# phantomzone-org/fhe-ram

Measured on AMD Instinct MI355X. Metric: encrypted RAM read ops/s + write ops/s at 2^18 entries; achieved HBM GB/s vs peak, higher is better.
Workload: dtype f64

## Files before the change

fhe-ram_amd/csrc/ctx.hpp:

```cpp
#pragma once
#include "../../include/fheram.h"
#include "kernels.hpp"
#include "cmux_chain.hpp"

#include <algorithm>
#include <atomic>
#include <cstdio>
#include <cstdlib>
#include <cstring>
#include <map>
#include <string>
#include <vector>

using namespace fk;

namespace {

thread_local std::string g_create_err;


struct ProfCls {
    uint64_t launches = 0, blocks = 0;
    double ms = 0.0;
    std::vector<std::pair<hipEvent_t, hipEvent_t>> pending;
// ... 128 lines not shown
    unsigned* h_mid_fb = nullptr;
    unsigned* d_mid_sync[2] = {nullptr, nullptr};
    double* d_mid_big[2] = {nullptr, nullptr};
    double* d_mid_y[2] = {nullptr, nullptr};
    uint64_t inv_id[2] = {0, 0};
    double* d_prep_inv = nullptr;
    int32_t* d_ggsw_inv = nullptr;
    hipEvent_t ev_inv[2] = {nullptr, nullptr};
    bool inv_pending[2] = {false, false};
    hipEvent_t ev_wdone = nullptr;
    bool wdone_pending = false;
    hipEvent_t ev_opstart = nullptr;
    bool opstart_valid = false;
    bool wide_unsynced = false;
    bool derive_unsynced = false;
    int32_t* h_pin[2] = {nullptr, nullptr};
    hipEvent_t ev_pin[2] = {nullptr, nullptr};
    int64_t* h_res = nullptr;
    int64_t* d_h_res = nullptr;
    int32_t* h_w = nullptr;
    hipEvent_t ev_w = nullptr;
    bool w_busy = false;
    bool side_begun = false;
    bool trhi_in_C = false;
    bool tree_rotate_pending = false;
    bool words_staged = false;
    int profile = 0;
    std::map<std::string, ProfCls> prof;
    std::vector<hipEvent_t> ev_pool;
    hipEvent_t t0 = nullptr, t1 = nullptr;
// ... 33 lines not shown
}
int check_precision(fheram_ctx* c) {
    if (c->h_ro_flag && __atomic_load_n(c->h_ro_flag, __ATOMIC_RELAXED))
        return fail(c, FHERAM_ERR_PRECISION, "FP64 round-off of an inverse transform exceeded 3/8 (fheram_roundoff_max): the rounded integers are no longer trustworthy");
    return FHERAM_OK;
}
#define HIPCHK(c, call)                                                                     \
    do {                                                                                    \
        hipError_t e_ = (call);                                                             \
        if (e_ != hipSuccess)                                                               \
            return fail((c), FHERAM_ERR_DEVICE, std::string(#call) + ": " + hipGetErrorString(e_)); \
    } while (0)

GlweRef ref(int32_t* p, long sy, long sx) { return GlweRef{p, sy, sx}; }

hipEvent_t get_event(fheram_ctx* c) {
    if (!c->ev_pool.empty()) { hipEvent_t e = c->ev_pool.back(); c->ev_pool.pop_back(); return e; }
    hipEvent_t e = nullptr; c->res.event(&e, true); return e;
}
struct ProfScope {
    fheram_ctx* c; ProfCls* cls = nullptr; hipEvent_t a = nullptr;
    ProfScope(fheram_ctx* c_, const char* name, uint64_t blocks, int steps = 1) : c(c_) {
        if (!c->profile) return;
        if (c->profile == 2 && !strstr(name, "chain_launch")) return;
        cls = &c->prof[name];
        cls->launches += steps; cls->blocks += blocks * steps;
        a = get_event(c);
        hipEventRecord(a, c->cur);
    }
    ~ProfScope() {
// ... 78 lines not shown
            HIPCHK(c, hipMemcpyAsync(c->h_pin[k & 1], src + off, m * sizeof(int32_t), hipMemcpyDeviceToHost, c->stream));
            HIPCHK(c, hipEventRecord(c->ev_pin[k & 1], c->stream));
        }
        if (k > 0) {
            const size_t off = (k - 1) * PIN_CHUNK, m = std::min(PIN_CHUNK, n - off);
            HIPCHK(c, hipEventSynchronize(c->ev_pin[(k - 1) & 1]));
            widen(c->h_pin[(k - 1) & 1], dst + off, m);
        }
    }
    return FHERAM_OK;
}
int stage_words(fheram_ctx* c, int32_t* d_w, const int64_t* w, int n_ct) {
    if (c->w_busy) { HIPCHK(c, hipEventSynchronize(c->ev_w)); c->w_busy = false; }
    const size_t n = (size_t)n_ct * fheram_ctx::GLWE;
    if (!narrow(w, c->h_w, n)) return fail(c, FHERAM_ERR_RANGE, "limb out of the normalised range [-2^16, 2^16]");
    HIPCHK(c, hipMemcpyAsync(d_w, c->h_w, n * sizeof(int32_t), hipMemcpyHostToDevice, c->stream));
    HIPCHK(c, hipEventRecord(c->ev_w, c->stream));
    c->w_busy = true;
    return FHERAM_OK;
}

}
```

fhe-ram_amd/csrc/fheram.hip:

```cpp
#include <unistd.h>
#include <atomic>
#include "path.hpp"

extern "C" {

int fheram_params_default(fheram_params* p) {
    if (!p) return FHERAM_ERR_INVALID_ARG;
    std::memset(p, 0, sizeof(*p));
    p->log_n = 12; p->base2k = 17; p->rank = 1;
    p->k_glwe_pt = 3; p->k_glwe_ct = 51; p->k_ggsw_addr = 68; p->k_evk_trace = 68; p->k_evk_ggsw_inv = 85;
    p->word_size = 4; p->n_decomp = 4;
    p->decomp_n[0] = p->decomp_n[1] = p->decomp_n[2] = p->decomp_n[3] = 3;
    p->max_addr = (uint64_t)1 << 14;
    return FHERAM_OK;
}

const char* fheram_last_error(const fheram_ctx* c) { return c ? c->err.c_str() : g_create_err.c_str(); }

void fheram_config_default(fheram_config* cfg) {
    if (!cfg) return;
    fheram_config d = config_builtin();
    auto env = [](const char* n) { const char* v = getenv(n); return (v && v[0]) ? v[0] : '\0'; };
    if (env("FHERAM_LIMB_SPLIT") == '0') d.limb_split = 0;
    if (env("FHERAM_FINE_SPLIT") == '0') d.fine_split = 0;
// ... 322 lines not shown
    return result_export(c, &run, 1, c->h_res, c->d_h_res, nullptr);
}
int fheram_result_download(fheram_ctx* c, int64_t* out) {
    if (!c || !out) return FHERAM_ERR_INVALID_ARG;
    const int64_t* src = nullptr;
    const int rc = fheram_result_map(c, &src);
    if (rc != FHERAM_OK) return rc;
    std::memcpy(out, src, (size_t)c->ws * fheram_ctx::GLWE * sizeof(int64_t));
    return FHERAM_OK;
}
int fheram_sync(fheram_ctx* c) {
    if (!c) return FHERAM_ERR_INVALID_ARG;
    HIPCHK(c, hipSetDevice(c->device));
    HIPCHK(c, hipStreamSynchronize(c->stream));
    HIPCHK(c, hipGetLastError());
    c->wide_unsynced = c->derive_unsynced = false;
    return check_precision(c);
}
int fheram_roundoff_max(fheram_ctx* c, double* max_out) {
    if (!c || !max_out) return FHERAM_ERR_INVALID_ARG;
    HIPCHK(c, hipSetDevice(c->device));
    HIPCHK(c, hipStreamSynchronize(c->stream));
    HIPCHK(c, hipStreamSynchronize(c->stream2));
    double m = 0.0;
    HIPCHK(c, hipMemcpy(&m, c->d_tw + N, sizeof(double), hipMemcpyDeviceToHost));
    *max_out = m;
    if (c->cfg.monitor && m > MON_LIMIT) __atomic_store_n(c->h_ro_flag, 1u, __ATOMIC_RELAXED);
    return check_precision(c);
}
int fheram_roundoff_reset(fheram_ctx* c) {
    if (!c) return FHERAM_ERR_INVALID_ARG;
// ... 72 lines not shown
    if (w) { rc = fheram_word_stage(c, w, n_w); if (rc != FHERAM_OK) { write_side_abort(c); return rc; } }
    rc = run_op(c, addr, 2, [&] {
        if (!c->side_begun) write_side_begin(o, ctx_view(c));
        int r2 = write_top(o, ctx_view(c));
        return r2 == FHERAM_OK ? write_rows(o, ctx_view(c)) : r2;
    });
    if (rc != FHERAM_OK) return rc;
    c->ram.state = false;
    HIPCHK(c, hipGetLastError());
    return FHERAM_OK;
}

namespace {
int export_glwes(fheram_ctx* c, const int32_t* src, void* dst, int on_device, size_t n_glwe) {
    const size_t n = n_glwe * fheram_ctx::GLWE;
    if (on_device) { HIPCHK(c, hipMemcpyAsync(dst, src, n * 4, hipMemcpyDeviceToDevice, c->stream)); return FHERAM_OK; }
    return download_i64(c, (int64_t*)dst, src, n);
}
int import_glwes(fheram_ctx* c, int32_t* dst, const void* src, int on_device, size_t n_glwe) {
    const size_t n = n_glwe * fheram_ctx::GLWE;
    if (on_device) { HIPCHK(c, hipMemcpyAsync(dst, src, n * 4, hipMemcpyDeviceToDevice, c->stream)); return FHERAM_OK; }
    return upload_i64(c, dst, (const int64_t*)src, n);
}
}

int fheram_shard_info(const fheram_ctx* c, int* shard, int* n_shards, size_t* local_rows) {
    if (!c) return FHERAM_ERR_INVALID_ARG;
    if (shard) *shard = c->shard;
    if (n_shards) *n_shards = c->n_shards;
    if (local_rows) *local_rows = c->rows;
    return FHERAM_OK;
}
int fheram_read_partial(fheram_ctx* c, const fheram_addr* addr, int prepare_write, void* out, int out_on_device) {
    int rc = check_common(c, addr);
    if (rc != FHERAM_OK) return rc;
    if (!out) return fail(c, FHERAM_ERR_INVALID_ARG, "null output");
    if (c->ram.state) return fail(c, FHERAM_ERR_STATE, "invalid call to Memory.read: internal state is true -> requires calling Memory.write");
    HIPCHK(c, hipSetDevice(c->device));
    GlweRef packed;
    rc = read_local(one_addr(c, &addr), ctx_view(c), prepare_write != 0, &packed, true);
    if (rc != FHERAM_OK) return rc;
    HIPCHK(c, hipGetLastError());
    if (prepare_write) c->ram.state = true;
    return export_glwes(c, c->d_part, out, out_on_device, (size_t)c->ws);
}
int fheram_stream_signal(fheram_ctx* c, void* hip_stream) {
    if (!c) return FHERAM_ERR_INVALID_ARG;
    HIPCHK(c, hipSetDevice(c->device));
    HIPCHK(c, hipEventRecord(c->ev_xout, c->stream));
    HIPCHK(c, hipStreamWaitEvent((hipStream_t)hip_stream, c->ev_xout, 0));
    return FHERAM_OK;
}
int fheram_stream_wait(fheram_ctx* c, void* hip_stream) {
    if (!c) return FHERAM_ERR_INVALID_ARG;
    HIPCHK(c, hipSetDevice(c->device));
    HIPCHK(c, hipEventRecord(c->ev_xin, (hipStream_t)hip_stream));
    HIPCHK(c, hipStreamWaitEvent(c->stream, c->ev_xin, 0));
    return FHERAM_OK;
}
int fheram_device_malloc(fheram_ctx* c, size_t bytes, void** out) {
    if (!c || !out || bytes == 0) return fail(c, FHERAM_ERR_INVALID_ARG, "bad argument");
    HIPCHK(c, hipSetDevice(c->device));
    HIPCHK(c, hipMalloc(out, bytes));
    return FHERAM_OK;
}
int fheram_device_free(fheram_ctx* c, void* ptr) {
    if (!c) return FHERAM_ERR_INVALID_ARG;
    HIPCHK(c, hipSetDevice(c->device));
    HIPCHK(c, hipFree(ptr));
    return FHERAM_OK;
}
// ... 143 lines not shown
    return download_i64(c, ggsw_out, c->d_ggsw_tmp, fheram_ctx::GGSW);
}

int fheram_timer_begin(fheram_ctx* c) {
    if (!c) return FHERAM_ERR_INVALID_ARG;
    HIPCHK(c, hipSetDevice(c->device));
    HIPCHK(c, hipEventRecord(c->t0, c->stream));
    return FHERAM_OK;
}
int fheram_timer_end(fheram_ctx* c, float* ms) {
    if (!c || !ms) return FHERAM_ERR_INVALID_ARG;
    HIPCHK(c, hipSetDevice(c->device));
    HIPCHK(c, hipEventRecord(c->t1, c->stream));
    HIPCHK(c, hipEventSynchronize(c->t1));
    HIPCHK(c, hipEventElapsedTime(ms, c->t0, c->t1));
    c->wide_unsynced = c->derive_unsynced = false;
    return check_precision(c);
}
int fheram_profile_enable(fheram_ctx* c, int on) {
    if (!c) return FHERAM_ERR_INVALID_ARG;
    c->profile = on == 2 ? 2 : (on != 0);
    return FHERAM_OK;
}
int fheram_profile_reset(fheram_ctx* c) {
    if (!c) return FHERAM_ERR_INVALID_ARG;
    hipSetDevice(c->device);
    prof_collect(c);
    c->prof.clear();
    return FHERAM_OK;
}
int fheram_profile_get(fheram_ctx* c, const char* cls, uint64_t* launches, uint64_t* blocks, double* total_ms) {
// ... 133 lines not shown
```

fhe-ram_amd/csrc/kernels.hpp:

```cpp
#pragma once
#include "../../include/fheram.h"
#include "fft_dev.hpp"
#include <type_traits>

namespace fk {

#ifdef FK_STAMP
__device__ unsigned long long g_stamps[192];
#define STAMP(i)                                                                                   \
    do {                                                                                           \
        __builtin_amdgcn_sched_barrier(0);                                                         \
        if (threadIdx.x == 0 && blockIdx.x == 0 && blockIdx.y == 0 && blockIdx.z == 0) {           \
            unsigned long long t_;                                                                 \
            asm volatile("s_memtime %0\n\ts_waitcnt lgkmcnt(0)" : "=s"(t_)::"memory");            \
            g_stamps[i] = t_;                                                                      \
        }                                                                                          \
        __builtin_amdgcn_sched_barrier(0);                                                         \
    } while (0)
#define STAMPZ(i)                                                                                  \
    do {                                                                                           \
        __builtin_amdgcn_sched_barrier(0);                                                         \
        if (threadIdx.x == 0 && blockIdx.x == 0 && blockIdx.y == 0 && (blockIdx.z == 0 || blockIdx.z == 3)) { \
            unsigned long long t_;                                                                 \
            asm volatile("s_memtime %0\n\ts_waitcnt lgkmcnt(0)" : "=s"(t_)::"memory");            \
// ... 164 lines not shown
__device__ __forceinline__ void load_ops_p(OpRegs& o, const double* __restrict__ g, int tid) {
#ifdef FK_NO_PROLOGUE_OPS
#pragma unroll
    for (int kk = 0; kk < E / 2; kk++) asm volatile("" : "=v"(o.v[kk].x), "=v"(o.v[kk].y));
#else
    load_ops(o, g, tid);
#endif
}
__device__ __forceinline__ void mac_regs(double (&acc)[E], const double (&x)[E], const OpRegs& o) {
#pragma unroll
    for (int kk = 0; kk < E / 2; kk++) cmac(acc[2 * kk], acc[2 * kk + 1], x[2 * kk], x[2 * kk + 1], o.v[kk].x, o.v[kk].y);
}

constexpr int BF = 3, BI = 1;
#ifndef FK_CHAIN_VGPRS
#define FK_CHAIN_VGPRS 120
#endif
#define FK_WIDE_VGPRS 128
static_assert(BF <= BMAX && BI <= BMAX, "LDS holds BMAX exchange buffers");

template <int S, int R = 0>
__device__ __forceinline__ void fwd_all(double (&x)[S][E], const double* tw, double* data, int tid) {
    if constexpr (R < S) {
        constexpr int C = (S - R < BF) ? (S - R) : BF;
        ntt_fwd<C>(*reinterpret_cast<double(*)[C][E]>(&x[R]), tw, data, tid);
        fwd_all<S, R + C>(x, tw, data, tid);
    }
}

template <int SA, int SG>
__device__ __forceinline__ void ep_mac(double (&acc)[E], const double (&x0)[SA][E], const double (&x1)[SA][E], OpRegs (&g)[SA],
// ... 1196 lines not shown
        const double d1 = take_digit(r_);
        int dst = tid + T * k + ka.t;
        const bool ng = dst >= N;
        if (ng) dst -= N;
        gstore_i32(op + glwe_off(2, co), (unsigned)dst * 4u, cneg((int)d2, ng));
        gstore_i32(op + glwe_off(1, co), (unsigned)dst * 4u, cneg((int)d1, ng));
        gstore_i32(op + glwe_off(0, co), (unsigned)dst * 4u, cneg((int)r_, ng));
    }
}

struct RowChainArgs {
    EpChainArgs ep;
    KsChainArgs ks;
    GlweRef hi, trhi;
    int store_ep = 0;
};
#define FK_READ_CHAIN_ARGS RowChainArgs
#define FK_READ_CHAIN_TABLE 0
#define FK_KS_CHAIN_NAME k_keyswitch_chain
#define FK_READ_CHAIN_NAME k_read_chain
#define FK_VG FK_CHAIN_VGPRS
#include "chain_kernels.inc"
#undef FK_KS_CHAIN_NAME
#undef FK_READ_CHAIN_NAME
#undef FK_VG
#define FK_KS_CHAIN_NAME k_keyswitch_chain_w
#define FK_READ_CHAIN_NAME k_read_chain_w
#define FK_VG FK_WIDE_VGPRS
#include "chain_kernels.inc"
#undef FK_KS_CHAIN_NAME
// ... 803 lines not shown
```

fhe-ram_amd/csrc/launch.hpp:

```cpp
#pragma once
#include "ctx.hpp"

namespace {

template <typename F>
void with_evk(const fheram_ctx* c, F&& f) {
    if (c->s_evk == 5) f(std::integral_constant<int, 5>{});
    else f(std::integral_constant<int, 4>{});
}
template <typename F>
void with_evk_wide(fheram_ctx* c, bool wide, F&& f) {
    if (wide) c->wide_unsynced = true;
    with_evk(c, [&](auto sk) { if (wide) f(sk, std::true_type{}); else f(sk, std::false_type{}); });
}
bool capturing(const fheram_ctx* c) { return c->cfg.graph && !c->profile; }

constexpr int LIMB_SPLIT_MAX = 64;
constexpr int EW_SLICES = 8;
int pick_nco(const fheram_ctx* c, int gx, int gy, bool one_wg = false) {
    if (c->cfg.nco != 0) return c->cfg.nco;
    if (one_wg) return 2;
    return ((long)gx * gy * 2 <= c->cus) ? 1 : 2;
}
void launch_prepare(fheram_ctx* c, const int32_t* in, double* out, int npoly, int64_t gal = 0) {
// ... 16 lines not shown
        hipLaunchKernelGGL((k_ext_product_fine_norm<3, 4>), dim3(gx, gy, 2 * (N / 256)), dim3(256), 0, c->cur, res, big_of(c));
        return;
    }
    if (use_limb_split(c, gx, gy, 4)) {
        hipLaunchKernelGGL((k_ext_product<3, 4, 1, 1>), dim3(gx, gy, 8), dim3(T), LDS_BYTES, c->cur, a, res, ggsw, c->d_tw, big_of(c));
        hipLaunchKernelGGL((k_ext_product<3, 4, 1, 2>), dim3(gx, gy, 2), dim3(T), 0, c->cur, a, res, ggsw, c->d_tw, big_of(c));
        return;
    }
    if (pick_nco(c, gx, gy) == 1) hipLaunchKernelGGL((k_ext_product<3, 4, 1>), dim3(gx, gy, 2), dim3(T), LDS_BYTES, c->cur, a, res, ggsw, c->d_tw, big_of(c));
    else {
        ProfScope pf(c, "ext_product_fused", (uint64_t)gx * gy);
        hipLaunchKernelGGL((k_ext_product<3, 4, 2>), dim3(gx, gy, 1), dim3(T), LDS_BYTES, c->cur, a, res, ggsw, c->d_tw, big_of(c));
    }
}
template <int MODE, int SX, int SK, int SO>
void launch_ks(fheram_ctx* c, const KsArgs& ka, int gx, int gy) {
    if (gx <= 0 || gy <= 0) return;
    ProfScope ps(c, "keyswitch", (uint64_t)gx * gy);
    if (use_fine_split(c, gx, gy, 2 * SK * SX)) {
        KsArgs kb = ka;
        kb.big = big_of(c);
        hipLaunchKernelGGL((k_keyswitch_fine<MODE, SX, SK>), dim3(gx, gy, 2 * SK * SX), dim3(T), LDS_BYTES, c->cur, kb);
        hipLaunchKernelGGL((k_keyswitch_norm<MODE, SX, SK, SO, SX>), dim3(gx, gy, 2 * (N / 256)), dim3(256), 0, c->cur, kb);
        return;
    }
    if (use_limb_split(c, gx, gy, SK)) {
        KsArgs kb = ka;
        kb.big = big_of(c);
        hipLaunchKernelGGL((k_keyswitch<MODE, SX, SK, SO, 1, 1>), dim3(gx, gy, 2 * SK), dim3(T), LDS_BYTES, c->cur, kb);
        hipLaunchKernelGGL((k_keyswitch_norm<MODE, SX, SK, SO>), dim3(gx, gy, 2 * (N / 256)), dim3(256), 0, c->cur, kb);
        return;
    }
    constexpr bool FUSABLE = (SX == 3) && (MODE != KS_PAIR);
    if constexpr (MODE == KS_PAIR && SX == 3 && SO == 3) {
        if (c->cfg.pair_z) {
            hipLaunchKernelGGL((k_pair_z<SK>), dim3(gx, gy, 2), dim3(T), LDS_BYTES, c->cur, ka);
            return;
        }
    }
    if (!FUSABLE || pick_nco(c, gx, gy) == 1) {
        hipLaunchKernelGGL((k_keyswitch<MODE, SX, SK, SO, 1>), dim3(gx, gy, 2), dim3(T), LDS_BYTES, c->cur, ka);
// ... 212 lines not shown
    ra.hi = dst; ra.trhi = dst;
    if (t.ws > 0) {
        c->wide_unsynced = true;
        with_evk(c, [&](auto sk) {
            constexpr int SK = decltype(sk)::value;
            hipLaunchKernelGGL((k_read_chain_t<SK, 4>), dim3(gx, gy, 1), dim3(T), LDS_BYTES, c->cur, with_table(ra, t));
        });
        return;
    }
    with_evk_wide(c, c->wide, [&](auto sk, auto w) {
        constexpr int SK = decltype(sk)::value;
        if constexpr (decltype(w)::value) hipLaunchKernelGGL((k_read_chain_w<SK, 4>), dim3(gx, gy, 1), dim3(T), LDS_BYTES, c->cur, ra);
        else hipLaunchKernelGGL((k_read_chain<SK, 4>), dim3(gx, gy, 1), dim3(T), LDS_BYTES, c->cur, ra);
    });
}
void launch_write_chain(fheram_ctx* c, GlweRef src, int rot_mul, int rot_base, GlweRef data, GlweRef trhi, const double* prep, int d, int n_tr, int gx, int gy, const OpndTable& t) {
    ProfScope ps(c, "write_chain_launch", (uint64_t)gx * gy, 1);
    RowChainArgs ra;
    fill_row_chain(c, ra, prep, d, 0, n_tr);
    ra.ks.base = ks_args(c, src, src, data, trace_key(c, 0), c->gal[0], 0, rot_mul, rot_base);
    ra.ks.buf[0] = ra.ks.buf[1] = data;
    ra.hi = data; ra.trhi = trhi;
    ra.ep.src = data; ra.ep.buf[0] = ra.ep.buf[1] = data;
    c->wide_unsynced = true;
    with_evk(c, [&](auto sk) {
        constexpr int SK = decltype(sk)::value;
        if (t.ws > 0) hipLaunchKernelGGL((k_write_chain_t<SK, 4>), dim3(gx, gy, 1), dim3(T), LDS_BYTES, c->cur, with_table(ra, t));
        else hipLaunchKernelGGL((k_write_chain<SK, 4>), dim3(gx, gy, 1), dim3(T), LDS_BYTES, c->cur, ra);
    });
}
void launch_trace_tail(fheram_ctx* c, GlweRef src, const GlweRef (&b)[2], int start, int n, int gx, int gy,
                       const double* prep = nullptr, int d = 0, GlweRef ep_out = GlweRef{nullptr, 0, 0}, bool store_ep = false, const OpndTable& t = {}) {
    ProfScope ps(c, "keyswitch", (uint64_t)gx * gy, n);
    ProfScope pt(c, "keyswitch_tail_launch", (uint64_t)gx * gy * n, 1);
    TailArgs ta;
    ta.src = src; ta.buf[0] = b[0]; ta.buf[1] = b[1]; ta.tw = c->d_tw; ta.big = big_of(c); ta.sync = c->d_tail_sync;
    ta.n_ep = prep ? d : 0; ta.ep_out = ep_out;
    for (int i = 0; i < TAIL_EP_MAX; i++) ta.ggsw[i] = (prep && i < d) ? prep + (size_t)i * fheram_ctx::GGSW : nullptr;
// ... 87 lines not shown
        }
        live = std::min<size_t>(live, (size_t)h);
        cur = nxt;
    }
    return cur;
}
int coord_first_digit(const fheram_ctx* c, int ci) { int s = 0; for (int i = 0; i < ci; i++) s += (int)c->base2d[i].size(); return s; }
double* digits_of(const fheram_ctx* c, double* table, int ci) { return table + (size_t)coord_first_digit(c, ci) * fheram_ctx::GGSW; }
void coordinate_prepare(fheram_ctx* c, const fheram_addr* addr, int ci, double* table) {
    const int d = (int)c->base2d[ci].size();
    launch_prepare(c, addr->d_ggsw + (size_t)coord_first_digit(c, ci) * fheram_ctx::GGSW, digits_of(c, table, ci), d * (int)(fheram_ctx::GGSW / N));
}
void coordinate_prepare_all(fheram_ctx* c, const fheram_addr* addr, double* table) {
    launch_prepare(c, addr->d_ggsw, table, c->n_digits * (int)(fheram_ctx::GGSW / N));
}
void ggsw_inverse(fheram_ctx* c, const int32_t* in, int32_t* tmp, int d) {
    const long g4 = (long)fheram_ctx::GLWE4;
    int32_t* inp = const_cast<int32_t*>(in);
    KsArgs ka = ks_args(c, ref(inp, (long)fheram_ctx::GGSW, 2 * g4), ref(inp, 0, 0), ref(tmp, (long)fheram_ctx::GGSW, 2 * g4), c->d_atk_inv, -1);
    launch_ks<KS_AUTO, 4, 5, 4>(c, ka, fheram_ctx::DNUM_CT, d);
    KsArgs kt = ks_args(c, ref(tmp, (long)fheram_ctx::GGSW, 2 * g4), ref(tmp, 0, 0), ref(tmp + g4, (long)fheram_ctx::GGSW, 2 * g4), c->d_tsk, 1);
    launch_ks<KS_TENSOR, 4, 5, 4>(c, kt, fheram_ctx::DNUM_CT, d);
}
void coordinate_prepare_inv(fheram_ctx* c, const fheram_addr* addr, int ci, int32_t* tmp, double* prep) {
    const int d = (int)c->base2d[ci].size();
    ggsw_inverse(c, addr->d_ggsw + (size_t)coord_first_digit(c, ci) * fheram_ctx::GGSW, tmp, d);
    launch_prepare(c, tmp, prep, d * (int)(fheram_ctx::GGSW / N));
}

void precompute_inverse(fheram_ctx* c, const fheram_addr* addr, int ci, bool fork, unsigned gate_seq = 0) {
    if (fork && c->wdone_pending) {
        hipStreamWaitEvent(c->stream2, c->ev_wdone, 0);
        c->wdone_pending = false;
    }
    if (fork && gate_seq) {
        if (c->opstart_valid) { hipStreamWaitEvent(c->stream2, c->ev_opstart, 0); c->opstart_valid = false; }
        hipLaunchKernelGGL(k_tail_gate, dim3(1), dim3(64), 0, c->stream2, c->d_tail_sync + TAIL_GROUPS * 32 + 2, gate_seq);
    } else if (fork) {
        hipEventRecord(c->ev_fork, c->stream);
        hipStreamWaitEvent(c->stream2, c->ev_fork, 0);
    }
    hipStream_t keep = c->cur;
    c->cur = c->stream2;
    coordinate_prepare_inv(c, addr, ci, c->d_ggsw_inv + (size_t)coord_first_digit(c, ci) * fheram_ctx::GGSW, digits_of(c, c->d_prep_inv, ci));
    hipEventRecord(c->ev_inv[ci], c->stream2);
    c->cur = keep;
    c->inv_id[ci] = addr->id;
    c->inv_pending[ci] = true;
}
void wait_inverse(fheram_ctx* c, hipStream_t s, int ci) { if (!capturing(c)) hipStreamWaitEvent(s, c->ev_inv[ci], 0); }

}
```

fhe-ram_amd/csrc/path.hpp:

```cpp
#pragma once
#include "launch.hpp"

namespace {

struct Opnds {
    fheram_ctx* c;
    RamState* st;
    const fheram_addr* const* addrs;
    int n, ws;
    double *tab, *tab_inv;
    long stride;
    unsigned src_map;
    bool bank;
    int member(int k) const { return (int)((src_map >> (4 * k)) & 15u); }
    int Y() const { return n * ws; }
    double* prep(int k, int ci) const { return digits_of(c, tab + k * stride, ci); }
    double* inv(int k, int ci) const { return digits_of(c, tab_inv + k * stride, ci); }
    GlweRef slice(GlweRef r, int k) const { r.p += (long)k * ws * r.sy; return r; }
    GlweRef rows(GlweRef r, int k) const { return slice(r, member(k)); }
    OpndTable table() const { return n == 1 ? OpndTable{} : OpndTable{ws, stride, src_map}; }
    bool row_fuse(int d, int n_tr, int gx) const { return use_row_fuse(c, d, n_tr, gx, Y(), bank); }
};
Opnds one_addr(fheram_ctx* c, const fheram_addr* const* a, int ws, RamState* st) { return Opnds{c, st, a, 1, ws, c->d_prep, c->d_prep_inv, 0, 0, false}; }
Opnds one_addr(fheram_ctx* c, const fheram_addr* const* a) { return one_addr(c, a, c->ws, &c->ram); }
// ... 10 lines not shown
}

void read_local_done(const fheram_ctx* c, RamState* st, bool prepare_write) {
    if (c->n2 == 2) st->memo_alone = (prepare_write && c->cfg.memo) ? LOGN - ilog2_ceil(c->rows_glob) : 0;
}
void read_top_done(fheram_ctx* c, RamState* st, bool prepare_write) {
    st->memo_top = prepare_write && c->cfg.memo;
    st->res_in_trtop = st->memo_top;
    c->prep1_ready = false;
}
void write_done(fheram_ctx* c, RamState* st) { st->memo_top = false; st->memo_alone = 0; c->side_begun = false; c->tree_rotate_pending = false; }

template <typename F>
int run_op(fheram_ctx* c, const fheram_addr* addr, int which, F&& enqueue) {
    if (!capturing(c)) return enqueue();
    fheram_addr* a = const_cast<fheram_addr*>(addr);
    const unsigned sig = 1u | (c->ram.memo_top ? 2u : 0u) | ((unsigned)c->ram.memo_alone << 2) | (c->side_begun ? 64u : 0u) |
                         (c->inv_id[0] == addr->id ? 128u : 0u) | (c->inv_id[1] == addr->id ? 256u : 0u);
    if (a->graph[which] && a->graph_sig[which] != sig) { hipGraphExecDestroy(a->graph[which]); a->graph[which] = nullptr; }
    if (!a->graph[which]) {
        hipGraph_t g = nullptr;
        HIPCHK(c, hipStreamBeginCapture(c->stream, hipStreamCaptureModeThreadLocal));
        const int rc = enqueue();
        const hipError_t e = hipStreamEndCapture(c->stream, &g);
        if (rc != FHERAM_OK || e != hipSuccess) {
            if (g) hipGraphDestroy(g);
            return rc != FHERAM_OK ? rc : fail(c, FHERAM_ERR_DEVICE, std::string("hipStreamEndCapture: ") + hipGetErrorString(e));
        }
        const hipError_t e2 = hipGraphInstantiate(&a->graph[which], g, nullptr, nullptr, 0);
        hipGraphDestroy(g);
// ... 7 lines not shown
}

int check_common(fheram_ctx* c, const fheram_addr* addr) {
    if (!c) return FHERAM_ERR_INVALID_ARG;
    mid_rearm(c);
    if (!addr || addr->ctx != c) return fail(c, FHERAM_ERR_INVALID_ARG, "address does not belong to this context (layout mismatch, ram.rs:404)");
    if (addr->empty) return fail(c, FHERAM_ERR_INVALID_ARG, "empty address: fheram_address_alloc without fheram_address_derive");
    if (!c->ram.initialized) return fail(c, FHERAM_ERR_UNINITIALIZED, "unitialized memory: self.data.len()=0");
    if (!c->keys_loaded) return fail(c, FHERAM_ERR_KEYS, "evaluation keys not loaded");
    return FHERAM_OK;
}

int read_local(const Opnds& o, const RamView& a, bool prepare_write, GlweRef* packed_out, bool to_part) {
    fheram_ctx* c = o.c;
    const int n = o.n, ws = o.ws, Y = o.Y(), R = (int)c->rows;
    c->wide = !prepare_write || n > 1;
    if (n == 1 && prepare_write && c->cfg.pre_inv == 1 && !capturing(c) && (c->wide_unsynced || c->derive_unsynced)) {
        hipEventRecord(c->ev_opstart, c->stream);
        c->opstart_valid = true;
    }
    const long G = (long)fheram_ctx::GLWE;
    const long sy = (long)c->rows * G;
    GlweRef data = ref(a.rows, sy, G), A = ref(a.A, sy, G), B = ref(a.B, sy, G);
    GlweRef part = ref(a.part, G, 0);
    const bool all = (c->n_shards == 1 && c->n2 == 2);
    for (int k = 0; k < n; k++)
        if (all) coordinate_prepare_all(c, o.addrs[k], o.tab + k * o.stride); else coordinate_prepare(c, o.addrs[k], 0, o.tab + k * o.stride);
    c->prep1_ready = all;
    read_local_done(c, o.st, prepare_write);
    const int d0 = (int)c->base2d[0].size();
// ... 13 lines not shown
        launch_read_chain(c, data, prepare_write ? &data : nullptr, A, o.prep(0, 0), d0, L0, R, Y, o.table());
        packed = pack_levels(c, a.A, a.A, a.B, sy, G, (size_t)R, Y, 0, L0, keep, a.C, a.D);
    } else {
        for (int k = 0; k < n; k++)
            if (prepare_write) ep_chain(c, o.rows(data, k), o.rows(data, k), o.slice(A, k), o.prep(k, 0), d0, R, ws);
            else ep_chain(c, o.rows(data, k), o.slice(A, k), o.slice(B, k), o.prep(k, 0), d0, R, ws);
        packed = pack_levels(c, prepare_write ? a.rows : a.A, a.A, a.B, sy, G, (size_t)R, Y, L0, L0, keep, a.C, a.D);
    }
    *packed_out = ref(packed, sy, 0);
    if (to_part) launch_copy(c, *packed_out, part, 1, Y);
    return FHERAM_OK;
}
int read_top(const Opnds& o, const RamView& a, bool prepare_write, int32_t* gathered, GlweRef pk) {
    fheram_ctx* c = o.c;
    const int n = o.n, ws = o.ws, Y = o.Y();
    c->wide = !prepare_write || n > 1;
    const long G = (long)fheram_ctx::GLWE;
    GlweRef tmp = ref(a.tmp, G, 0);
    GlweRef last = pk;
    const int d1 = c->n2 == 2 ? (int)c->base2d[1].size() : 0;
    auto tail_top = [&] { return chain_form(c, ChainQuery{false, LOGN, 1, Y}).form == ChainForm::Tail; };
    const bool fuse_ep = c->n2 == 2 && c->cfg.tail_ep && d1 >= 2 && d1 <= TAIL_EP_MAX && tail_top();
    GlweRef ep_out = ref(prepare_write ? a.tree : a.tmp2, G, 0);
    auto products1 = [&] { for (int k = 0; k < n; k++) ep_chain(c, o.slice(pk, k), o.slice(ep_out, k), o.slice(tmp, k), o.prep(k, 1), d1, 1, ws); };
    if (c->n2 == 2) {
        if (gathered) {
            const int kG = ilog2_ceil((size_t)c->n_shards);
            int32_t* a0 = c->d_gat[1];
            int32_t* a1 = c->d_gat[2];
            int32_t* packed = pack_levels(c, gathered, a0, a1, G, (long)ws * G, (size_t)c->n_shards, ws, 0, LOGN - kG);
// ... 77 lines not shown
    return FHERAM_OK;
}
RamView reads_view(const fheram_ctx* c, const ReadBufs& L) { return RamView{c->d_data, L.A, L.B, L.C, nullptr, L.tmp2, L.tmp, L.tmp2, L.res, nullptr, nullptr, nullptr}; }

struct ResRun { const int32_t* src; size_t n; };
int result_export(fheram_ctx* c, const ResRun* runs, int n_runs, int64_t* h, int64_t* d_h, int64_t* out) {
    size_t n = 0;
    for (int i = 0; i < n_runs; i++) {
        const int n4 = (int)(runs[i].n / 4);
        hipLaunchKernelGGL(k_export_i64, dim3((n4 + 255) / 256), dim3(256), 0, c->stream, runs[i].src, reinterpret_cast<long long*>(d_h + n), n4,
                           reinterpret_cast<const long long*>(c->d_tw + N));
        n += runs[i].n;
    }
    HIPCHK(c, hipStreamSynchronize(c->stream));
    HIPCHK(c, hipGetLastError());
    c->wide_unsynced = c->derive_unsynced = false;
    double m;
    std::memcpy(&m, h + n, 8);
    if (c->cfg.monitor && m > MON_LIMIT) __atomic_store_n(c->h_ro_flag, 1u, __ATOMIC_RELAXED);
    const int rc = check_precision(c);
    if (rc == FHERAM_OK && out) std::memcpy(out, h, n * sizeof(int64_t));
    return rc;
}

int reads_export(fheram_ctx* c, const ReadBufs& L, size_t first, size_t n_ct, int64_t* out) {
    const ResRun run{L.res + first * fheram_ctx::GLWE, n_ct * fheram_ctx::GLWE};
    return result_export(c, &run, 1, L.h_res, L.d_h_res, out);
}
template <typename F>
int read_many(fheram_ctx* c, ReadBufs& L, RamState* st, const fheram_addr* const* addrs, int n, int ws, unsigned src_map, bool bank, int64_t* out, F&& kept) {
    int rc = reads_reserve(c, L, n, ws);
    if (rc != FHERAM_OK) return rc;
    const Opnds o = table_opnds(c, st, addrs, n, ws, L.prep, nullptr, src_map, bank);
    rc = read_impl(o, reads_view(c, L), false);
    if (rc != FHERAM_OK) return rc;
    kept(o);
    HIPCHK(c, hipGetLastError());
    return out ? reads_export(c, L, 0, (size_t)n * ws, out) : FHERAM_OK;
}

int write_top(const Opnds& o, const RamView& v) {
    fheram_ctx* c = o.c;
    c->wide = true;
    const long G = (long)fheram_ctx::GLWE;
    const long sy = (long)c->rows * G;
    const int n = o.n, ws = o.ws, Y = o.Y();
    GlweRef wref = ref(v.w, G, 0), tmp = ref(v.tmp, G, 0), tmp2 = ref(v.tmp2, G, 0), tree = ref(v.tree, G, 0);
    GlweRef top = (c->n2 != 1) ? tree : ref(v.rows, sy, 0);
    GlweRef tr = tmp;
    if (o.st->memo_top) tr = ref(v.trtop, G, 0);
    else trace_steps(c, top, tmp, tmp2, 0, LOGN, 1, Y);
    {
        ProfScope ps(c, "elementwise", Y);
        hipLaunchKernelGGL((k_sub_add_norm<3>), dim3(1, Y, EW_SLICES), dim3(256), 0, c->cur, top, tr, wref, top);
    }
    o.st->memo_top = false;
    if (c->n2 == 2) {
// ... 2 lines not shown
            if (n == 1 && c->inv_pending[1]) wait_inverse(c, c->stream, 1);
            for (int k = 0; k < n; k++) coordinate_prepare_inv(c, o.addrs[k], 1, c->d_ggsw_tmp, o.inv(k, 1));
        }
        if (n == 1) { c->inv_pending[1] = false; c->inv_id[1] = 0; }
        for (int k = 0; k < n; k++)
            ep_chain(c, o.slice(tree, k), o.slice(ref(v.part, G, 0), k), o.slice(tmp, k), o.inv(k, 1), (int)c->base2d[1].size(), 1, ws);
        c->tree_rotate_pending = true;
    }
    return FHERAM_OK;
}
void write_side_begin(const Opnds& o, const RamView& v) {
    fheram_ctx* c = o.c;
    c->wide = true;
    const long G = (long)fheram_ctx::GLWE;
    const long sy = (long)c->rows * G;
    hipEventRecord(c->ev_fork, c->stream);
    hipStreamWaitEvent(c->stream2, c->ev_fork, 0);
    c->cur = c->stream2;
    if (c->n2 == 2) {
        const int kept = o.st->memo_alone;
        c->trhi_in_C = kept > 0 && (LOGN - kept) % 2 == 1;
        if (kept > 0) trace_steps(c, ref(v.A, sy, G), ref(c->trhi_in_C ? v.C : v.A, sy, G), ref(c->trhi_in_C ? v.A : v.C, sy, G), kept, LOGN, (int)c->rows, o.Y());
        else trace_steps(c, ref(v.rows, sy, G), ref(v.A, sy, G), ref(v.C, sy, G), 0, LOGN, (int)c->rows, o.Y());
        o.st->memo_alone = 0;
    }
    if (o.n == 1 && c->inv_id[0] == o.addrs[0]->id) wait_inverse(c, c->stream2, 0);
    else for (int k = 0; k < o.n; k++) coordinate_prepare_inv(c, o.addrs[k], 0, c->d_ggsw_tmp2, o.inv(k, 0));
    if (o.n == 1) { c->inv_id[0] = 0; c->inv_pending[0] = false; }
    hipEventRecord(c->ev_join, c->stream2);
    c->cur = c->stream;
    c->side_begun = true;
}
void write_side_abort(fheram_ctx* c) {
    if (!c->side_begun) return;
    hipStreamWaitEvent(c->stream, c->ev_join, 0);
    c->side_begun = false;
}
int write_rows(const Opnds& o, const RamView& v) {
    fheram_ctx* c = o.c;
    c->wide = true;
    const long G = (long)fheram_ctx::GLWE;
    const long sy = (long)c->rows * G;
    const int n = o.n, ws = o.ws, Y = o.Y(), R = (int)c->rows;
    GlweRef data = ref(v.rows, sy, G), A = ref(v.A, sy, G), B = ref(v.B, sy, G), D = ref(v.D, sy, G);
    GlweRef trhi = ref(c->trhi_in_C ? v.C : v.A, sy, G), part = ref(v.part, G, 0);
    const int d0 = (int)c->base2d[0].size();
    const bool fuse = c->n2 == 2 && o.row_fuse(d0, LOGN, R);
    if (fuse) {
        hipStreamWaitEvent(c->stream, c->ev_join, 0);
        launch_write_chain(c, part, c->n_shards, c->shard, data, trhi, o.inv(0, 0), d0, LOGN, R, Y, o.table());
    } else if (c->n2 == 2)
        trace_steps(c, part, B, D, 0, LOGN, R, Y, c->n_shards, c->shard);
    if (c->tree_rotate_pending) {
        ProfScope ps(c, "elementwise", Y);
        hipLaunchKernelGGL((k_rotate<3>), dim3(1, Y, EW_SLICES), dim3(256), 0, c->cur, part, ref(v.tree, G, 0), -(int)c->rows_glob);
    }
    if (!fuse) {
        hipStreamWaitEvent(c->stream, c->ev_join, 0);
        if (c->n2 == 2) {
            ProfScope ps(c, "elementwise", (uint64_t)R * Y);
            hipLaunchKernelGGL((k_sub_add_norm<3>), dim3(R, Y, EW_SLICES), dim3(256), 0, c->cur, data, trhi, B, data);
        }
        for (int k = 0; k < n; k++) ep_chain(c, o.slice(data, k), o.slice(data, k), o.slice(A, k), o.inv(k, 0), d0, R, ws);
    }
    if (n == 1 && !capturing(c)) { hipEventRecord(c->ev_wdone, c->stream); c->wdone_pending = true; }
    write_done(c, o.st);
    o.st->state = false;
    return FHERAM_OK;
// ... 4 lines not shown
```

fhe-ram_amd/csrc/setup.hpp:

```cpp
#pragma once
#include "launch.hpp"

namespace {
void wipe_free(hipStream_t st, void* d, size_t bytes) {
    if (!d) return;
    if (hipMemsetAsync(d, 0, bytes, st) == hipSuccess) hipStreamSynchronize(st);
    hipFree(d);
}
void wipe_host(void* p, size_t bytes) {
    volatile unsigned char* v = static_cast<volatile unsigned char*>(p);
    for (size_t i = 0; i < bytes; i++) v[i] = 0;
}
}

namespace {

constexpr int64_t NOISE_LIM = (int64_t)1 << 30;
int noise_limb(int k) { return (k + BASE2K - 1) / BASE2K - 1; }

template <int S, int DEC>
void launch_enc(fheram_ctx* c, int32_t* cts, const double* s_hat, const int32_t* pt1, int n) {
    ProfScope ps(c, "encrypt", (uint64_t)n);
    hipLaunchKernelGGL((k_encrypt_sk<S, DEC>), dim3(n), dim3(T), LDS_BYTES, c->cur, cts, s_hat, c->d_tw, pt1);
}
// ... 506 lines not shown
        ca.fu[k] = fus[k]->d_prep;
        ca.out[k] = addrs[k]->d_ggsw;
        for (int ci = 0; ci < 2; ci++) if (c->inv_pending[ci] && c->inv_id[ci] == addrs[k]->id) wait_inv[ci] = true;
    }
    for (int ci = 0; ci < 2; ci++) if (wait_inv[ci]) HIPCHK(c, hipStreamWaitEvent(c->stream, c->ev_inv[ci], 0));
    if (c->side_begun) HIPCHK(c, hipStreamWaitEvent(c->stream, c->ev_join, 0));
    c->cur = c->stream;
    {
        const int rows = fheram_ctx::DNUM_CT * 2;
        ProfScope ps(c, "derive", (uint64_t)n * c->n_digits * rows);
        cmux_chain_launch(dim3(rows, c->n_digits, n), c->cur, ca);
    }
    HIPCHK(c, hipGetLastError());
    for (int k = 0; k < n; k++) { addrs[k]->id = next_addr_id(); addrs[k]->empty = false; }
    c->derive_unsynced = true;
    return FHERAM_OK;
}

}
```

fhe-ram_amd/csrc/write_chain.inc:

```
#if FK_WRITE_CHAIN_TABLE
#define FK_WC_OPND(i) (ra.ep.ggsw[i] + table_opnd_offset(ra))
#else
#define FK_WC_OPND(i) ra.ep.ggsw[i]
#endif
template <int SK, int SG>
__global__ __launch_bounds__(T, T / 256) __attribute__((amdgpu_num_vgpr(FK_WIDE_VGPRS))) void FK_WRITE_CHAIN_NAME(FK_WRITE_CHAIN_ARGS ra) {
    extern __shared__ __attribute__((aligned(16))) double lds[];
    RoMonitor ro_mon(lds, ra.ep.tw);
    double vc[E];
    KsArgs ka = ra.ks.base;
#pragma unroll 1
    for (int i = 0; i < ra.ks.n; i++) {
        ka.out = ra.ks.buf[i & 1];
        ka.key = ra.ks.key[i];
        ka.ginv = ra.ks.ginv[i];
        int tid = vt((int)threadIdx.x);
        asm volatile("" : "+v"(tid));
        __builtin_assume(tid >= 0 && tid < T);
        if (i == 0) ks_trace_l<SK, false, 1>(ka, lds, true, tid, vc);
        else if (i + 1 < ra.ks.n) ks_trace_l<SK, true, 1>(ka, lds, false, tid, vc);
        else { ka.b = ra.hi; ka.out = ra.trhi; ks_trace_l<SK, true, 2>(ka, lds, false, tid, vc); }
        ka.rot_mul = 0;
        ka.rot_base = 0;
    }
// ... 15 lines not shown
```

Before: 1309.

## Skip redundant stream fork when idle, fold tree rotate into write chain

Tracks whether the main stream is known idle after a host sync and, if so, skips the event-record/wait fork onto the side stream for single-shard writes. The tree rotation kernel is fused into the write chain's first block row, removing a separate elementwise launch. Side-stream ggsw inverse keyswitches avoid the fine/limb-split variants, and the chain VGPR budget is raised slightly. The idle flag must be cleared at every enqueue point, which risks a missed dependency if one site is overlooked.

```diff
diff --git a/fhe-ram_amd/csrc/ctx.hpp b/fhe-ram_amd/csrc/ctx.hpp
--- a/fhe-ram_amd/csrc/ctx.hpp
+++ b/fhe-ram_amd/csrc/ctx.hpp
@@ -166,6 +166,7 @@
     bool opstart_valid = false;
     bool wide_unsynced = false;
     bool derive_unsynced = false;
+    bool main_idle = false;
     int32_t* h_pin[2] = {nullptr, nullptr};
     hipEvent_t ev_pin[2] = {nullptr, nullptr};
     int64_t* h_res = nullptr;
@@ -229,6 +230,9 @@
 
 GlweRef ref(int32_t* p, long sy, long sx) { return GlweRef{p, sy, sx}; }
 
+void main_waited(fheram_ctx* c) { c->wide_unsynced = c->derive_unsynced = false; c->main_idle = true; }
+void main_enqueued(fheram_ctx* c) { c->main_idle = false; }
+
 hipEvent_t get_event(fheram_ctx* c) {
     if (!c->ev_pool.empty()) { hipEvent_t e = c->ev_pool.back(); c->ev_pool.pop_back(); return e; }
     hipEvent_t e = nullptr; c->res.event(&e, true); return e;
@@ -337,6 +341,7 @@
     if (c->w_busy) { HIPCHK(c, hipEventSynchronize(c->ev_w)); c->w_busy = false; }
     const size_t n = (size_t)n_ct * fheram_ctx::GLWE;
     if (!narrow(w, c->h_w, n)) return fail(c, FHERAM_ERR_RANGE, "limb out of the normalised range [-2^16, 2^16]");
+    main_enqueued(c);
     HIPCHK(c, hipMemcpyAsync(d_w, c->h_w, n * sizeof(int32_t), hipMemcpyHostToDevice, c->stream));
     HIPCHK(c, hipEventRecord(c->ev_w, c->stream));
     c->w_busy = true;
diff --git a/fhe-ram_amd/csrc/fheram.hip b/fhe-ram_amd/csrc/fheram.hip
--- a/fhe-ram_amd/csrc/fheram.hip
+++ b/fhe-ram_amd/csrc/fheram.hip
@@ -360,7 +360,7 @@
     HIPCHK(c, hipSetDevice(c->device));
     HIPCHK(c, hipStreamSynchronize(c->stream));
     HIPCHK(c, hipGetLastError());
-    c->wide_unsynced = c->derive_unsynced = false;
+    main_waited(c);
     return check_precision(c);
 }
 int fheram_roundoff_max(fheram_ctx* c, double* max_out) {
@@ -463,12 +463,12 @@
 namespace {
 int export_glwes(fheram_ctx* c, const int32_t* src, void* dst, int on_device, size_t n_glwe) {
     const size_t n = n_glwe * fheram_ctx::GLWE;
-    if (on_device) { HIPCHK(c, hipMemcpyAsync(dst, src, n * 4, hipMemcpyDeviceToDevice, c->stream)); return FHERAM_OK; }
+    if (on_device) { main_enqueued(c); HIPCHK(c, hipMemcpyAsync(dst, src, n * 4, hipMemcpyDeviceToDevice, c->stream)); return FHERAM_OK; }
     return download_i64(c, (int64_t*)dst, src, n);
 }
 int import_glwes(fheram_ctx* c, int32_t* dst, const void* src, int on_device, size_t n_glwe) {
     const size_t n = n_glwe * fheram_ctx::GLWE;
-    if (on_device) { HIPCHK(c, hipMemcpyAsync(dst, src, n * 4, hipMemcpyDeviceToDevice, c->stream)); return FHERAM_OK; }
+    if (on_device) { main_enqueued(c); HIPCHK(c, hipMemcpyAsync(dst, src, n * 4, hipMemcpyDeviceToDevice, c->stream)); return FHERAM_OK; }
     return upload_i64(c, dst, (const int64_t*)src, n);
 }
 }
@@ -496,6 +496,7 @@
 int fheram_stream_signal(fheram_ctx* c, void* hip_stream) {
     if (!c) return FHERAM_ERR_INVALID_ARG;
     HIPCHK(c, hipSetDevice(c->device));
+    main_enqueued(c);
     HIPCHK(c, hipEventRecord(c->ev_xout, c->stream));
     HIPCHK(c, hipStreamWaitEvent((hipStream_t)hip_stream, c->ev_xout, 0));
     return FHERAM_OK;
@@ -504,6 +505,7 @@
     if (!c) return FHERAM_ERR_INVALID_ARG;
     HIPCHK(c, hipSetDevice(c->device));
     HIPCHK(c, hipEventRecord(c->ev_xin, (hipStream_t)hip_stream));
+    main_enqueued(c);
     HIPCHK(c, hipStreamWaitEvent(c->stream, c->ev_xin, 0));
     return FHERAM_OK;
 }
@@ -677,7 +679,7 @@
     HIPCHK(c, hipEventRecord(c->t1, c->stream));
     HIPCHK(c, hipEventSynchronize(c->t1));
     HIPCHK(c, hipEventElapsedTime(ms, c->t0, c->t1));
-    c->wide_unsynced = c->derive_unsynced = false;
+    main_waited(c);
     return check_precision(c);
 }
 int fheram_profile_enable(fheram_ctx* c, int on) {
diff --git a/fhe-ram_amd/csrc/kernels.hpp b/fhe-ram_amd/csrc/kernels.hpp
--- a/fhe-ram_amd/csrc/kernels.hpp
+++ b/fhe-ram_amd/csrc/kernels.hpp
@@ -202,7 +202,7 @@
 
 constexpr int BF = 3, BI = 1;
 #ifndef FK_CHAIN_VGPRS
-#define FK_CHAIN_VGPRS 120
+#define FK_CHAIN_VGPRS 124
 #endif
 #define FK_WIDE_VGPRS 128
 static_assert(BF <= BMAX && BI <= BMAX, "LDS holds BMAX exchange buffers");
@@ -1429,6 +1429,8 @@
     KsChainArgs ks;
     GlweRef hi, trhi;
     int store_ep = 0;
+    GlweRef tree = {nullptr, 0, 0};
+    int tree_rho = 0;
 };
 #define FK_READ_CHAIN_ARGS RowChainArgs
 #define FK_READ_CHAIN_TABLE 0
diff --git a/fhe-ram_amd/csrc/launch.hpp b/fhe-ram_amd/csrc/launch.hpp
--- a/fhe-ram_amd/csrc/launch.hpp
+++ b/fhe-ram_amd/csrc/launch.hpp
@@ -54,17 +54,17 @@
     }
 }
 template <int MODE, int SX, int SK, int SO>
-void launch_ks(fheram_ctx* c, const KsArgs& ka, int gx, int gy) {
+void launch_ks(fheram_ctx* c, const KsArgs& ka, int gx, int gy, bool beside = false) {
     if (gx <= 0 || gy <= 0) return;
     ProfScope ps(c, "keyswitch", (uint64_t)gx * gy);
-    if (use_fine_split(c, gx, gy, 2 * SK * SX)) {
+    if (!beside && use_fine_split(c, gx, gy, 2 * SK * SX)) {
         KsArgs kb = ka;
         kb.big = big_of(c);
         hipLaunchKernelGGL((k_keyswitch_fine<MODE, SX, SK>), dim3(gx, gy, 2 * SK * SX), dim3(T), LDS_BYTES, c->cur, kb);
         hipLaunchKernelGGL((k_keyswitch_norm<MODE, SX, SK, SO, SX>), dim3(gx, gy, 2 * (N / 256)), dim3(256), 0, c->cur, kb);
         return;
     }
-    if (use_limb_split(c, gx, gy, SK)) {
+    if (!beside && use_limb_split(c, gx, gy, SK)) {
         KsArgs kb = ka;
         kb.big = big_of(c);
         hipLaunchKernelGGL((k_keyswitch<MODE, SX, SK, SO, 1, 1>), dim3(gx, gy, 2 * SK), dim3(T), LDS_BYTES, c->cur, kb);
@@ -307,7 +307,8 @@
         else hipLaunchKernelGGL((k_read_chain<SK, 4>), dim3(gx, gy, 1), dim3(T), LDS_BYTES, c->cur, ra);
     });
 }
-void launch_write_chain(fheram_ctx* c, GlweRef src, int rot_mul, int rot_base, GlweRef data, GlweRef trhi, const double* prep, int d, int n_tr, int gx, int gy, const OpndTable& t) {
+void launch_write_chain(fheram_ctx* c, GlweRef src, int rot_mul, int rot_base, GlweRef data, GlweRef trhi, const double* prep, int d, int n_tr, int gx, int gy, const OpndTable& t,
+                        const GlweRef* tree = nullptr, int tree_rho = 0) {
     ProfScope ps(c, "write_chain_launch", (uint64_t)gx * gy, 1);
     RowChainArgs ra;
     fill_row_chain(c, ra, prep, d, 0, n_tr);
@@ -315,6 +316,7 @@
     ra.ks.buf[0] = ra.ks.buf[1] = data;
     ra.hi = data; ra.trhi = trhi;
     ra.ep.src = data; ra.ep.buf[0] = ra.ep.buf[1] = data;
+    if (tree) { ra.tree = *tree; ra.tree_rho = tree_rho; }
     c->wide_unsynced = true;
     with_evk(c, [&](auto sk) {
         constexpr int SK = decltype(sk)::value;
@@ -432,17 +434,17 @@
 void coordinate_prepare_all(fheram_ctx* c, const fheram_addr* addr, double* table) {
     launch_prepare(c, addr->d_ggsw, table, c->n_digits * (int)(fheram_ctx::GGSW / N));
 }
-void ggsw_inverse(fheram_ctx* c, const int32_t* in, int32_t* tmp, int d) {
+void ggsw_inverse(fheram_ctx* c, const int32_t* in, int32_t* tmp, int d, bool beside = false) {
     const long g4 = (long)fheram_ctx::GLWE4;
     int32_t* inp = const_cast<int32_t*>(in);
     KsArgs ka = ks_args(c, ref(inp, (long)fheram_ctx::GGSW, 2 * g4), ref(inp, 0, 0), ref(tmp, (long)fheram_ctx::GGSW, 2 * g4), c->d_atk_inv, -1);
-    launch_ks<KS_AUTO, 4, 5, 4>(c, ka, fheram_ctx::DNUM_CT, d);
+    launch_ks<KS_AUTO, 4, 5, 4>(c, ka, fheram_ctx::DNUM_CT, d, beside);
     KsArgs kt = ks_args(c, ref(tmp, (long)fheram_ctx::GGSW, 2 * g4), ref(tmp, 0, 0), ref(tmp + g4, (long)fheram_ctx::GGSW, 2 * g4), c->d_tsk, 1);
-    launch_ks<KS_TENSOR, 4, 5, 4>(c, kt, fheram_ctx::DNUM_CT, d);
-}
-void coordinate_prepare_inv(fheram_ctx* c, const fheram_addr* addr, int ci, int32_t* tmp, double* prep) {
+    launch_ks<KS_TENSOR, 4, 5, 4>(c, kt, fheram_ctx::DNUM_CT, d, beside);
+}
+void coordinate_prepare_inv(fheram_ctx* c, const fheram_addr* addr, int ci, int32_t* tmp, double* prep, bool beside = false) {
     const int d = (int)c->base2d[ci].size();
-    ggsw_inverse(c, addr->d_ggsw + (size_t)coord_first_digit(c, ci) * fheram_ctx::GGSW, tmp, d);
+    ggsw_inverse(c, addr->d_ggsw + (size_t)coord_first_digit(c, ci) * fheram_ctx::GGSW, tmp, d, beside);
     launch_prepare(c, tmp, prep, d * (int)(fheram_ctx::GGSW / N));
 }
 
@@ -460,7 +462,7 @@
     }
     hipStream_t keep = c->cur;
     c->cur = c->stream2;
-    coordinate_prepare_inv(c, addr, ci, c->d_ggsw_inv + (size_t)coord_first_digit(c, ci) * fheram_ctx::GGSW, digits_of(c, c->d_prep_inv, ci));
+    coordinate_prepare_inv(c, addr, ci, c->d_ggsw_inv + (size_t)coord_first_digit(c, ci) * fheram_ctx::GGSW, digits_of(c, c->d_prep_inv, ci), true);
     hipEventRecord(c->ev_inv[ci], c->stream2);
     c->cur = keep;
     c->inv_id[ci] = addr->id;
diff --git a/fhe-ram_amd/csrc/path.hpp b/fhe-ram_amd/csrc/path.hpp
--- a/fhe-ram_amd/csrc/path.hpp
+++ b/fhe-ram_amd/csrc/path.hpp
@@ -48,6 +48,7 @@
 template <typename F>
 int run_op(fheram_ctx* c, const fheram_addr* addr, int which, F&& enqueue) {
     if (!capturing(c)) return enqueue();
+    main_enqueued(c);
     fheram_addr* a = const_cast<fheram_addr*>(addr);
     const unsigned sig = 1u | (c->ram.memo_top ? 2u : 0u) | ((unsigned)c->ram.memo_alone << 2) | (c->side_begun ? 64u : 0u) |
                          (c->inv_id[0] == addr->id ? 128u : 0u) | (c->inv_id[1] == addr->id ? 256u : 0u);
@@ -85,6 +86,7 @@
 int read_local(const Opnds& o, const RamView& a, bool prepare_write, GlweRef* packed_out, bool to_part) {
     fheram_ctx* c = o.c;
     const int n = o.n, ws = o.ws, Y = o.Y(), R = (int)c->rows;
+    main_enqueued(c);
     c->wide = !prepare_write || n > 1;
     if (n == 1 && prepare_write && c->cfg.pre_inv == 1 && !capturing(c) && (c->wide_unsynced || c->derive_unsynced)) {
         hipEventRecord(c->ev_opstart, c->stream);
@@ -128,6 +130,7 @@
 int read_top(const Opnds& o, const RamView& a, bool prepare_write, int32_t* gathered, GlweRef pk) {
     fheram_ctx* c = o.c;
     const int n = o.n, ws = o.ws, Y = o.Y();
+    main_enqueued(c);
     c->wide = !prepare_write || n > 1;
     const long G = (long)fheram_ctx::GLWE;
     GlweRef tmp = ref(a.tmp, G, 0);
@@ -235,7 +238,7 @@
     }
     HIPCHK(c, hipStreamSynchronize(c->stream));
     HIPCHK(c, hipGetLastError());
-    c->wide_unsynced = c->derive_unsynced = false;
+    main_waited(c);
     double m;
     std::memcpy(&m, h + n, 8);
     if (c->cfg.monitor && m > MON_LIMIT) __atomic_store_n(c->h_ro_flag, 1u, __ATOMIC_RELAXED);
@@ -262,6 +265,7 @@
 
 int write_top(const Opnds& o, const RamView& v) {
     fheram_ctx* c = o.c;
+    main_enqueued(c);
     c->wide = true;
     const long G = (long)fheram_ctx::GLWE;
     const long sy = (long)c->rows * G;
@@ -294,8 +298,11 @@
     c->wide = true;
     const long G = (long)fheram_ctx::GLWE;
     const long sy = (long)c->rows * G;
-    hipEventRecord(c->ev_fork, c->stream);
-    hipStreamWaitEvent(c->stream2, c->ev_fork, 0);
+    if (!(c->main_idle && !capturing(c) && c->n_shards == 1)) {
+        hipEventRecord(c->ev_fork, c->stream);
+        hipStreamWaitEvent(c->stream2, c->ev_fork, 0);
+    }
+    main_enqueued(c);
     c->cur = c->stream2;
     if (c->n2 == 2) {
         const int kept = o.st->memo_alone;
@@ -318,6 +325,7 @@
 }
 int write_rows(const Opnds& o, const RamView& v) {
     fheram_ctx* c = o.c;
+    main_enqueued(c);
     c->wide = true;
     const long G = (long)fheram_ctx::GLWE;
     const long sy = (long)c->rows * G;
@@ -326,12 +334,14 @@
     GlweRef trhi = ref(c->trhi_in_C ? v.C : v.A, sy, G), part = ref(v.part, G, 0);
     const int d0 = (int)c->base2d[0].size();
     const bool fuse = c->n2 == 2 && o.row_fuse(d0, LOGN, R);
+    const bool rot_in_chain = fuse && c->tree_rotate_pending && c->n_shards == 1;
+    const GlweRef tree = ref(v.tree, G, 0);
     if (fuse) {
         hipStreamWaitEvent(c->stream, c->ev_join, 0);
-        launch_write_chain(c, part, c->n_shards, c->shard, data, trhi, o.inv(0, 0), d0, LOGN, R, Y, o.table());
+        launch_write_chain(c, part, c->n_shards, c->shard, data, trhi, o.inv(0, 0), d0, LOGN, R, Y, o.table(), rot_in_chain ? &tree : nullptr, -(int)c->rows_glob);
     } else if (c->n2 == 2)
         trace_steps(c, part, B, D, 0, LOGN, R, Y, c->n_shards, c->shard);
-    if (c->tree_rotate_pending) {
+    if (c->tree_rotate_pending && !rot_in_chain) {
         ProfScope ps(c, "elementwise", Y);
         hipLaunchKernelGGL((k_rotate<3>), dim3(1, Y, EW_SLICES), dim3(256), 0, c->cur, part, ref(v.tree, G, 0), -(int)c->rows_glob);
     }
diff --git a/fhe-ram_amd/csrc/setup.hpp b/fhe-ram_amd/csrc/setup.hpp
--- a/fhe-ram_amd/csrc/setup.hpp
+++ b/fhe-ram_amd/csrc/setup.hpp
@@ -544,7 +544,8 @@
     HIPCHK(c, hipGetLastError());
     for (int k = 0; k < n; k++) { addrs[k]->id = next_addr_id(); addrs[k]->empty = false; }
     c->derive_unsynced = true;
-    return FHERAM_OK;
-}
-
-}
+    main_enqueued(c);
+    return FHERAM_OK;
+}
+
+}
diff --git a/fhe-ram_amd/csrc/write_chain.inc b/fhe-ram_amd/csrc/write_chain.inc
--- a/fhe-ram_amd/csrc/write_chain.inc
+++ b/fhe-ram_amd/csrc/write_chain.inc
@@ -8,6 +8,17 @@
     extern __shared__ __attribute__((aligned(16))) double lds[];
     RoMonitor ro_mon(lds, ra.ep.tw);
     double vc[E];
+    if (ra.tree.p != nullptr && blockIdx.x == 0) {
+        const int32_t* ap = at(ra.ks.base.a);
+        int32_t* op = at(ra.tree);
+        for (int idx = (int)threadIdx.x; idx < 2 * N; idx += T) {
+            const int col = idx >> LOGN, i = idx & (N - 1);
+            int src; bool sgn;
+            rot_src(i, ra.tree_rho, src, sgn);
+#pragma unroll
+            for (int j = 0; j < 3; j++) op[glwe_off(j, col) + i] = cneg(ap[glwe_off(j, col) + src], sgn);
+        }
+    }
     KsArgs ka = ra.ks.base;
 #pragma unroll 1
     for (int i = 0; i < ra.ks.n; i++) {
```

After: 1328, median of 6. +1.5%, better.
